# Christopher-Wang/DistriFlow

Measured on AMD Instinct MI355X. Metric: images/sec (whole node), MNIST CNN sync-SGD at 1/2/4/8 MI355X; async speedup, higher is better.
Workload: dtype bf16; 1 GPU; model=lenet5, global_batch=4096, per_gpu_batch=4096, parallelism=dp1, optimizer=sgd, graph=full, steps_per_graph=64, p2p_reason=single rank, step=train+reduce/update, params=61706

## Files before the change

csrc/bindings_fused.cpp:

```cpp
#include "bindings_comm.h"

namespace dfa_py {
namespace {

struct CPIn {
  const void* x = nullptr;
  int u8 = 0;
  const long long* idx = nullptr;
  long long nrows = 0;
};

CPIn cp_input(const torch::Tensor& x, const c10::optional<torch::Tensor>& idx, int64_t B, int64_t HWC) {
  CPIn r;
  TORCH_CHECK(x.is_cuda() && x.is_contiguous(), "x must be a contiguous GPU tensor");
  if (has(idx)) {
    need(*idx, at::kLong, "idx");
    TORCH_CHECK(idx->numel() >= B, "idx shorter than the batch");
    TORCH_CHECK(x.scalar_type() == at::kByte || x.scalar_type() == at::kBFloat16, "dataset must be u8 or bf16");
    TORCH_CHECK(x.dim() >= 1 && x.size(0) > 0 && x.numel() / x.size(0) == HWC, "dataset row size mismatch");
    TORCH_CHECK(x.scalar_type() == at::kByte, "indexed input must be a uint8 dataset");
    r.u8 = 1;
    r.idx = reinterpret_cast<const long long*>(idx->data_ptr<int64_t>());
    r.nrows = x.size(0);
  } else {
// ... 362 lines not shown
  need(labels, at::kInt, "lenet labels");
  TORCH_CHECK(labels.numel() >= (a.idx ? 1 : B), "lenet: labels too small");
  if (a.idx) a.nrows = std::min<int64_t>(a.nrows, labels.numel());
  a.labels = labels.data_ptr<int>();
  a.scale = (float)scale;
  const int64_t conv_n[4] = {150, 6, 2400, 16};
  for (int k = 0; k < 4; ++k) {
    need(conv[k], at::kFloat, "lenet conv param");
    need(conv_grads[k], at::kFloat, "lenet conv grad");
    TORCH_CHECK(conv[k].numel() == conv_n[k] && conv_grads[k].numel() == conv_n[k], "lenet: conv param size");
  }
  a.w1 = conv[0].data_ptr<float>();
  a.b1 = conv[1].data_ptr<float>();
  a.w2 = conv[2].data_ptr<float>();
  a.b2 = conv[3].data_ptr<float>();
  const int64_t NK[3][2] = {{120, 400}, {84, 120}, {10, 84}};
  const float* dw[3];
  const float* db[3];
  for (int l = 0; l < 3; ++l) {
    need(dense_w[l], at::kFloat, "lenet dense w");
    need(dense_b[l], at::kFloat, "lenet dense b");
    TORCH_CHECK(dense_w[l].numel() == NK[l][0] * NK[l][1], "lenet: dense ", l, " kernel must be [", NK[l][0], "][",
                NK[l][1], "]");
    TORCH_CHECK(dense_b[l].numel() == NK[l][0], "lenet: dense bias size");
    need(dense_gw[l], at::kFloat, "lenet dense gw");
    need(dense_gb[l], at::kFloat, "lenet dense gb");
    TORCH_CHECK(dense_gw[l].numel() == NK[l][0] * NK[l][1] && dense_gb[l].numel() == NK[l][0],
                "lenet: dense grad size");
    need(hT[l], at::kBFloat16, "lenet hT");
    need(dzT[l], at::kBFloat16, "lenet dzT");
    TORCH_CHECK(hT[l].dim() == 2 && hT[l].size(0) >= (NK[l][1] + 15) / 16 * 16 && hT[l].size(1) == lds,
                "lenet: hT must be [>= round16(K)][ldt]");
    TORCH_CHECK(dzT[l].dim() == 2 && dzT[l].size(0) >= (NK[l][0] + 15) / 16 * 16 && dzT[l].size(1) == lds,
                "lenet: dzT must be [>= round16(N)][ldt]");
    dw[l] = dense_w[l].data_ptr<float>();
    db[l] = dense_b[l].data_ptr<float>();
  }
  a.d1m = dw[0]; a.d2m = dw[1]; a.d3m = dw[2];
  a.d1b = db[0]; a.d2b = db[1]; a.d3b = db[2];
  const int nblk = dfa::lenet_blocks((int)B);
  need(conv_part, at::kFloat, "lenet conv_part");
  need(loss_part, at::kFloat, "lenet loss_part");
  need(stats, at::kFloat, "lenet stats");
  TORCH_CHECK(conv_part.numel() >= (int64_t)dfa::kLeNetConvStride * nblk, "lenet: conv_part too small");
  TORCH_CHECK(loss_part.numel() >= 2 * nblk && stats.numel() >= 2, "lenet: loss buffers too small");
  a.conv_part = conv_part.data_ptr<float>();
  a.loss_part = loss_part.data_ptr<float>();
  auto bp = [](torch::Tensor& t) { return reinterpret_cast<dfa::bf16*>(t.data_ptr()); };
  a.h0T = bp(hT[0]); a.h1T = bp(hT[1]); a.h2T = bp(hT[2]);
  a.dz1T = bp(dzT[0]); a.dz2T = bp(dzT[1]); a.dz3T = bp(dzT[2]);
  TORCH_CHECK(frag.is_cuda() && frag.is_contiguous() && (size_t)frag.nbytes() >= dfa::lenet_frag_bytes(),
              "lenet: fragment buffer too small");
  TORCH_CHECK(ftab.is_cuda() && ftab.scalar_type() == at::kByte && ftab.numel() == 98 * 2 * 16, "lenet: ftab");
  TORCH_CHECK(pxtab.is_cuda() && pxtab.scalar_type() == at::kShort && pxtab.numel() == 832, "lenet: pxtab");
  a.frag = frag.data_ptr();
  a.prep = prep ? 1 : 0;
  a.ftab = ftab.data_ptr<uint8_t>();
  a.pxtab = reinterpret_cast<const unsigned short*>(pxtab.data_ptr());
  a.B = (int)B;
  a.ldt = (int)lds;
  a.grad_scale = (float)grad_scale;
  dfa::LeNetRedArgs r{};
  r.kcols = (int)ldt;
  need(dense_part, at::kFloat, "lenet dense_part");
  TORCH_CHECK(dense_part.numel() >= dfa::lenet_dense_part_floats((int)B),
              "lenet: dense_part must hold lenet_dense_part_floats(B) zero-initialised floats");
  dfa::lenet_red_bind_scratch(dense_part.data_ptr<float>(), r);
  r.succ = red_succ ? 1 : 0;
  r.conv_part = a.conv_part;
  r.loss_part = a.loss_part;
  r.stats = stats.data_ptr<float>();
  r.g_w1 = conv_grads[0].data_ptr<float>();
  r.g_b1 = conv_grads[1].data_ptr<float>();
  r.g_w2 = conv_grads[2].data_ptr<float>();
  r.g_b2 = conv_grads[3].data_ptr<float>();
  for (int l = 0; l < 3; ++l) {
    r.L[l].dzT = reinterpret_cast<const dfa::bf16*>(dzT[l].data_ptr());
    r.L[l].hT = reinterpret_cast<const dfa::bf16*>(hT[l].data_ptr());
    r.L[l].gw = dense_gw[l].data_ptr<float>();
    r.L[l].gb = dense_gb[l].data_ptr<float>();
    r.L[l].N = (int)NK[l][0];
    r.L[l].K = (int)NK[l][1];
  }
  r.w1 = a.w1;
  r.w2 = a.w2;
  if (has(snap)) {
    need(*snap, at::kFloat, "lenet snap");
    TORCH_CHECK(snap->numel() >= 2 * 2550, "lenet: snap must hold 2 x 2550 floats");
    r.snap = snap->data_ptr<float>();
    TORCH_CHECK(conv_mom.empty() || conv_mom.size() == 2, "lenet: conv_mom = [m1, m2] or []");
    if (conv_mom.size() == 2) {
      need(conv_mom[0], at::kFloat, "lenet m1");
      need(conv_mom[1], at::kFloat, "lenet m2");
      TORCH_CHECK(conv_mom[0].numel() == 150 && conv_mom[1].numel() == 2400, "lenet: conv momentum sizes");
      r.m1 = conv_mom[0].data_ptr<float>();
      r.m2 = conv_mom[1].data_ptr<float>();
    }
  }
  if (has(sgd_master)) {
    need(*sgd_master, at::kFloat, "lenet sgd master");
    TORCH_CHECK(sgd_wbf.has_value() && sgd_hyper.has_value() && sgd_descs.has_value(),
                "lenet sgd: wbf, hyper and descs are required");
    need(*sgd_wbf, at::kBFloat16, "lenet sgd wbf");
    need(*sgd_hyper, at::kFloat, "lenet sgd hyper");
    TORCH_CHECK(sgd_hyper->numel() >= 5, "lenet sgd: hyper size");
    const torch::Tensor& dh = *sgd_descs;
    TORCH_CHECK(!dh.is_cuda() && dh.scalar_type() == at::kLong && dh.is_contiguous() &&
// ... 280 lines not shown
```

csrc/lenet_fused.hip:

```cpp
#include "common.h"
#include "diag.h"
#include "kernels.h"
#include "lenet_frag.h"
#include "ll_exchange.h"
#include "optim_device.h"
#include "ps_device.h"

#include <algorithm>
#include <cstdlib>
#include <type_traits>
#include <vector>

namespace dfa {
namespace {

constexpr int IMG = 8;
constexpr int NT = 512;
constexpr int NW = NT / 64;
constexpr int ccdiv(int a, int b) { return (a + b - 1) / b; }
constexpr int XS_ELEMS = IMG * 1024 + 32;
constexpr int OFF_XS = 0;
constexpr int OFF_P1 = OFF_XS + XS_ELEMS * 2;
constexpr int OFF_C1 = OFF_P1 + IMG * 196 * 16;
constexpr int DC2_RS = 104;
constexpr int NM = IMG * DC2_RS;
constexpr int OFF_K = OFF_C1 + IMG * 196 * 4;
constexpr int OFF_PX = OFF_K + 32;
constexpr int OFF_FT = OFF_PX + NM * 2;
constexpr int OFF_W = OFF_FT + 98 * 2 * 16;
constexpr int OFF_KZ = OFF_W + 128;
constexpr int OFF_U = OFF_KZ + 32;
constexpr int OFF_XS1 = OFF_U + 32;
constexpr int LD0 = 424, LD1 = 136, LD2 = 104, LD3 = 40;
constexpr int OFF_H0 = OFF_U;
constexpr int OFF_H1 = OFF_H0 + IMG * LD0 * 2;
constexpr int OFF_H2 = OFF_H1 + IMG * LD1 * 2;
constexpr int OFF_Z3 = OFF_H2 + IMG * LD2 * 2;
constexpr int OFF_Z2 = OFF_Z3 + IMG * LD3 * 2;
constexpr int OFF_Z1 = OFF_Z2 + IMG * LD2 * 2;
constexpr int OFF_ZR = OFF_Z1 + IMG * LD1 * 2;
constexpr int OFF_LG = OFF_ZR + LD0 * 2;
constexpr int OFF_C2 = OFF_LG + IMG * 16 * 4;
constexpr int U_DENSE = OFF_C2 + IMG * 25 * 16 - OFF_U;
constexpr int OFF_DC2 = OFF_U;
constexpr int U_DC2 = NM * 16 * 2;
constexpr int OFF_RED = OFF_XS1 + XS_ELEMS * 2;
constexpr int U_G = 32 + XS_ELEMS * 2 + 4 * 16 * 32 * 4;
__device__ __forceinline__ int dc2_swz(int t) { return t ^ ((t >> 3) & 7); }
constexpr int cmax(int a, int b) { return a > b ? a : b; }
constexpr int NFP1 = (FR_C2 - FR_C1) * 64, NFP2 = (FR_DG - FR_C2) * 64;
constexpr int OFF_FC1 = OFF_XS1;
constexpr int OFF_FC2 = OFF_U + U_DENSE;
constexpr int U_FC2 = U_DENSE + NFP2 * 16;
static_assert(FR_C1 == 0 && FR_C2 - FR_C1 == 15 && FR_DG - FR_C2 == 7, "phase 0 stages fragments 0 .. 21 as one range");
static_assert(OFF_FC1 + NFP1 * 16 <= OFF_XS1 + (XS_ELEMS / 8 - 1) * 16, "build_shift1 overwrites the conv1 fragments");
constexpr int OFF_DB = OFF_U + (cmax(cmax(cmax(U_DENSE, U_DC2), U_G), U_FC2) + 15) / 16 * 16;
constexpr int OFF_ST = OFF_DB + 864;
constexpr int LDS_BYTES = OFF_ST + 128;
static_assert(OFF_U == OFF_C1 + IMG * 196 * 4 + 128 + 98 * 2 * 16 + 800 * 2 + 128 && OFF_U % 16 == 0 && OFF_KZ % 16 == 0 && OFF_H1 % 16 == 0 && OFF_ZR % 16 == 0 && OFF_C2 % 16 == 0 && OFF_RED % 16 == 0 && OFF_DB % 16 == 0 && OFF_ST % 16 == 0 &&
                  OFF_PX % 16 == 0 && OFF_W % 16 == 0 && OFF_FC1 % 16 == 0 && OFF_FC2 % 16 == 0,
              "LDS carve must stay 16-byte aligned");
static_assert(2 * LDS_BYTES <= 160 * 1024, "two workgroups per CU");

typedef __bf16 bf16x4_vs __attribute__((__vector_size__(8)));

#define LN_STAMP(slot)                                                            \
  do {                                                                            \
    if (stamps) {                                                                 \
      __builtin_amdgcn_sched_barrier(0);                                          \
      unsigned long long t_;                                                      \
      asm volatile("s_memtime %0\n\ts_waitcnt lgkmcnt(0)" : "=s"(t_)::"memory"); \
      __builtin_amdgcn_sched_barrier(0);                                          \
      if (threadIdx.x == 0) STMP[(slot)] = t_;                                    \
    }                                                                             \
  } while (0)

template <int CTRL>
__device__ __forceinline__ float dpp_f(float v) {
  return __builtin_bit_cast(float, __builtin_amdgcn_update_dpp(0, __builtin_bit_cast(int, v), CTRL, 0xf, 0xf, false));
}
__device__ __forceinline__ float row16_max(float v) {
  v = fmaxf(v, dpp_f<0xB1>(v));
  v = fmaxf(v, dpp_f<0x4E>(v));
  v = fmaxf(v, dpp_f<0x141>(v));
  return fmaxf(v, dpp_f<0x140>(v));
}
__device__ __forceinline__ float row16_sum(float v) {
  v += dpp_f<0xB1>(v);
  v += dpp_f<0x4E>(v);
  v += dpp_f<0x141>(v);
  return v + dpp_f<0x140>(v);
}

__device__ __forceinline__ bf16x4 tr_read(const bf16* p) {
  auto* lp = (__attribute__((address_space(3))) bf16*)(const_cast<bf16*>(p));
  const bf16x4_vs v =
      __builtin_amdgcn_ds_read_tr16_b64_v4bf16(reinterpret_cast<__attribute__((address_space(3))) bf16x4_vs*>(lp));
  return __builtin_bit_cast(bf16x4, v);
}
__device__ __forceinline__ bf16x8 cat8(bf16x4 a, bf16x4 b) {
  bf16x8 r;
#pragma unroll
  for (int e = 0; e < 4; ++e) {
    r[e] = a[e];
    r[e + 4] = b[e];
  }
  return r;
}
__device__ __forceinline__ bf16x8 ld8(const bf16* p) { return *reinterpret_cast<const bf16x8*>(p); }
__device__ __forceinline__ void st8(bf16* p, const bf16x8& v) { *reinterpret_cast<bf16x8*>(p) = v; }
__device__ __forceinline__ bf16x8 zero8() {
// ... 130 lines not shown
    if (__hip_atomic_compare_exchange_strong(p.dlock + k, &free_, (unsigned)p.rank + 1u, __ATOMIC_RELAXED,
                                             __ATOMIC_RELAXED, __HIP_MEMORY_SCOPE_SYSTEM)) {
      P = __hip_atomic_load(p.pref + k, __ATOMIC_RELAXED, __HIP_MEMORY_SCOPE_SYSTEM);
      const unsigned* fl = ps_inbox_flags(p, k);
      while (n < R && n < 255u &&
             __hip_atomic_load(const_cast<unsigned*>(fl) + (P + n) % R, __ATOMIC_RELAXED, __HIP_MEMORY_SCOPE_SYSTEM) ==
                 P + n + 1u)
        ++n;
      if (n == 0) __hip_atomic_store(p.dlock + k, 0u, __ATOMIC_RELAXED, __HIP_MEMORY_SCOPE_SYSTEM);
      c = P + n;
    }
    __hip_atomic_store(ps_owner_drain_words(p) + k, ps_owner_word(ep, n, P), __ATOMIC_RELAXED, __HIP_MEMORY_SCOPE_AGENT);
    s_cnt[k] = c;
  }
  __syncthreads();
  if (threadIdx.x == 0) {
    unsigned cnt = 0xffffffffu;
    for (int j = 0; j < p.nshards; ++j) cnt = s_cnt[j] < cnt ? s_cnt[j] : cnt;
    const unsigned dec = __hip_atomic_load(p.scratch + kPSDecision, __ATOMIC_RELAXED, __HIP_MEMORY_SCOPE_AGENT) & 7u;
    if (dec == kPSAccept && cnt == p.scratch[kPSSeq]) cnt += 1u;
    if (dec == kPSAccept || dec == kPSReject) ps_note_refresh(p, cnt);
  }
}

__device__ __forceinline__ void lenet_ps_admission(const PSArgs& p, bool excl) {
  const long long bid = *p.bid_out;
  const unsigned applied0 = ps_read_applied(p);
  const unsigned ep = __hip_atomic_load(p.scratch + kPSEpoch, __ATOMIC_RELAXED, __HIP_MEMORY_SCOPE_AGENT) + 1u;
  const unsigned dec = ps_admit(p, false);
  const bool owner = p.owner_ring > 0;
  if (!owner && (dec == kPSAccept || dec == kPSReject)) ps_note_refresh(p, applied0 + (dec == kPSAccept ? 1u : 0u));
  __hip_atomic_store(p.scratch + kPSDecision, (ep << 3) | dec, __ATOMIC_RELAXED, __HIP_MEMORY_SCOPE_AGENT);
  if (excl) {
    __hip_atomic_store(p.scratch + kPSEpoch, ep, __ATOMIC_RELAXED, __HIP_MEMORY_SCOPE_AGENT);
    if (dec == kPSAccept) ps_publish_applied(p);
  }
  if (dec == kPSAccept && p.done_epoch != nullptr) complete_microbatch(p, bid);
}

template <bool TRIM>
__global__ void __launch_bounds__(NT, 2 * NT / 256) lenet_train_kernel(LeNetArgs a) {
  if ((int)blockIdx.x >= a.nblk) {
    if (a.ps_admit && threadIdx.x == 0) lenet_ps_admission(a.ps, a.ps_excl != 0);
    return;
  }
  extern __shared__ __attribute__((aligned(16))) char smem[];
  bf16* Xs = reinterpret_cast<bf16*>(smem + OFF_XS);
  bf16* Xs1 = reinterpret_cast<bf16*>(smem + OFF_XS1);
  bf16* P1 = reinterpret_cast<bf16*>(smem + OFF_P1);
  unsigned* C1 = reinterpret_cast<unsigned*>(smem + OFF_C1);
  bf16* KO = reinterpret_cast<bf16*>(smem + OFF_K);
  unsigned char* FT = reinterpret_cast<unsigned char*>(smem + OFF_FT);
  unsigned short* PX = reinterpret_cast<unsigned short*>(smem + OFF_PX);
  float* WS = reinterpret_cast<float*>(smem + OFF_W);
  bf16* H0 = reinterpret_cast<bf16*>(smem + OFF_H0);
  bf16* H1 = reinterpret_cast<bf16*>(smem + OFF_H1);
  bf16* H2 = reinterpret_cast<bf16*>(smem + OFF_H2);
  bf16* Z3 = reinterpret_cast<bf16*>(smem + OFF_Z3);
  bf16* Z2 = reinterpret_cast<bf16*>(smem + OFF_Z2);
  bf16* Z1 = reinterpret_cast<bf16*>(smem + OFF_Z1);
  bf16* ZR = reinterpret_cast<bf16*>(smem + OFF_ZR);
  float* LG = reinterpret_cast<float*>(smem + OFF_LG);
  unsigned char* C2 = reinterpret_cast<unsigned char*>(smem + OFF_C2);
  bf16* DC2 = reinterpret_cast<bf16*>(smem + OFF_DC2);
  float* RED = reinterpret_cast<float*>(smem + OFF_RED);

  const int tid = threadIdx.x, lane = tid & 63, w = __builtin_amdgcn_readfirstlane(tid >> 6), i = lane & 15,
            g = lane >> 4;
  const int r0 = lenet_img_group(blockIdx.x, a.nblk) * (TRIM ? a.ipw : IMG);
  const int rows = min(TRIM ? a.ipw : IMG, a.B - r0);
  const int nA = TRIM ? 2 * ((7 * rows + 1) / 2) : 56;
  const int nB = TRIM ? (13 * rows + 1) / 2 : NM / 16;
  const int nE = TRIM ? (13 * rows + 3) / 4 : NM / 32;
  const int nF = TRIM ? (49 * rows + 7) / 8 : 49;
  const int nG = TRIM ? 14 * rows : IMG * 14;
  const bf16x8* __restrict__ frag = reinterpret_cast<const bf16x8*>(a.frag);
  float* part = a.conv_part + (long long)blockIdx.x * kLeNetConvStride;
  unsigned long long* const stamps = a.stamps;
  unsigned long long* const STMP = reinterpret_cast<unsigned long long*>(smem + OFF_ST);
  LN_STAMP(0);

  const int ximg = tid / 28, xrow = tid - 28 * (tid / 28);
  const bool xload = tid < IMG * 28 && ximg < rows;
  const bool lload = tid >= 256 && tid < 256 + IMG && tid - 256 < rows;
  long long xsrc = 0, lsrc = 0;
  if (xload) xsrc = a.idx ? a.idx[r0 + ximg] : (long long)(r0 + ximg);
  if (lload) lsrc = a.idx ? a.idx[r0 + tid - 256] : (long long)(r0 + tid - 256);
  uint4 tabv = {0u, 0u, 0u, 0u};
  if (tid < 98 * 2) tabv = reinterpret_cast<const uint4*>(a.ftab)[tid];
  else if (tid >= 264 && tid < 264 + NM / 8) tabv = reinterpret_cast<const uint4*>(a.pxtab)[tid - 264];
  static_assert(98 * 2 <= 256 && 264 + NM / 8 <= 448 && 448 + 22 <= NT, "phase 0 staging thread ranges");
  float biasv = 0.f, dbv = 0.f;
  if (tid >= 448 && tid < 448 + 22) biasv = *(tid < 454 ? a.b1 + (tid - 448) : a.b2 + (tid - 454));
  if (tid < 214) dbv = *(tid < 120 ? a.d1b + tid : (tid < 204 ? a.d2b + (tid - 120) : a.d3b + (tid - 204)));
  constexpr int NFK = ccdiv(NFP1 + NFP2, NT);
  bf16x8 fv[NFK];
#pragma unroll
  for (int k = 0; k < NFK; ++k) fv[k] = frag[FR_C1 * 64 + min(tid + NT * k, NFP1 + NFP2 - 1)];
  const int lbl = a.labels[lsrc < 0 ? 0 : (lsrc >= a.nrows ? a.nrows - 1 : lsrc)];
  unsigned xv[14];
  {
    const long long src = xsrc < 0 ? 0 : (xsrc >= a.nrows ? a.nrows - 1 : xsrc);
    const int xr = xload ? xrow : 0;
    if (a.x_u8 != nullptr) {
      const unsigned* p = reinterpret_cast<const unsigned*>(a.x_u8 + src * 784 + xr * 28);
#pragma unroll
      for (int k = 0; k < 7; ++k) xv[k] = p[k];
    } else {
      const uint2* p = reinterpret_cast<const uint2*>(a.x_bf + src * 784 + xr * 28);
#pragma unroll
      for (int k = 0; k < 7; ++k) {
        const uint2 v = p[k];
        xv[2 * k] = v.x;
        xv[2 * k + 1] = v.y;
      }
    }
  }
  const bf16x8 z8 = zero8();
  bf16x8 one6 = z8;
  one6[6] = (bf16)1.f;
  for (int e = tid; e < (OFF_K - OFF_XS) / 16; e += NT)
    st8(Xs + 8 * e, (e >= OFF_P1 / 16 && e < OFF_C1 / 16) ? one6 : z8);
  static_assert(OFF_FC2 + NFP2 * 16 == OFF_DB, "the conv2 fragment image ends the union");
  if (tid < (OFF_FC1 - OFF_U) / 16) st8(reinterpret_cast<bf16*>(smem + OFF_U) + 8 * tid, z8);
  for (int e = (OFF_FC1 - OFF_U) / 16 + NFP1 + tid; e < (OFF_FC2 - OFF_U) / 16; e += NT)
    st8(reinterpret_cast<bf16*>(smem + OFF_U) + 8 * e, z8);
#pragma unroll
  for (int k = 0; k < NFK; ++k) {
    const int p = tid + NT * k;
    if (p < NFP1) st8(reinterpret_cast<bf16*>(smem + OFF_FC1) + 8 * p, fv[k]);
    else if (p < NFP1 + NFP2) st8(reinterpret_cast<bf16*>(smem + OFF_FC2) + 8 * (p - NFP1), fv[k]);
  }
  if (tid < 2) {
    bf16x8 o;
#pragma unroll
    for (int e = 0; e < 8; ++e) o[e] = (bf16)1.f;
    st8(KO + 8 * tid, o);
  } else if (tid < 4) {
    st8(reinterpret_cast<bf16*>(smem + OFF_KZ) + 8 * (tid - 2), z8);
  }
  if (tid < 98 * 2) reinterpret_cast<uint4*>(FT)[tid] = tabv;
  else if (tid >= 264 && tid < 264 + NM / 8) reinterpret_cast<uint4*>(PX)[tid - 264] = tabv;
  if (tid >= 448 && tid < 448 + 22) WS[tid - 448] = biasv;
  float* DB = reinterpret_cast<float*>(smem + OFF_DB);
  if (tid < 214) DB[tid] = dbv;
  int* LBL = reinterpret_cast<int*>(WS + 24);
  if (tid >= 256 && tid < 256 + IMG) LBL[tid - 256] = lbl;
  __syncthreads();
  bf16x8 bc[15];
#pragma unroll
  for (int f = 0; f < 15; ++f) bc[f] = ld8(reinterpret_cast<const bf16*>(smem + OFF_FC1) + 8 * (f * 64 + lane));
  if (xload) {
    unsigned* dst = reinterpret_cast<unsigned*>(Xs + ximg * 1024 + (xrow + 2) * 32 + 2);
    if (a.x_u8 != nullptr) {
#pragma unroll
      for (int k = 0; k < 7; ++k)
#pragma unroll
        for (int h = 0; h < 2; ++h) {
          const float f0 = (float)((xv[k] >> (16 * h)) & 255u) * a.scale;
          const float f1 = (float)((xv[k] >> (16 * h + 8)) & 255u) * a.scale;
          const unsigned lo = __builtin_bit_cast(unsigned short, f2bf(f0));
          const unsigned hi = __builtin_bit_cast(unsigned short, f2bf(f1));
          dst[2 * k + h] = lo | (hi << 16);
        }
    } else {
#pragma unroll
      for (int k = 0; k < 14; ++k) dst[k] = xv[k];
    }
  }
  __syncthreads();
  build_shift1(Xs, Xs1);
  __syncthreads();
  LN_STAMP(1);

  {
    const float b1c[3] = {WS[(i >> 3)], WS[2 + (i >> 3)], WS[4 + (i >> 3)]};
#pragma unroll 2
    for (int u = w; u < nA; u += NT / 64) {
      const int mt = u >> 1, x0 = (u & 1) * 16;
      const int m = 16 * mt + i;
      const int img = m / 56, rem = m - 56 * (m / 56);
      const bf16* abase = ((rem & 1) ? Xs1 : Xs) + img * 1024 + (rem >> 1) * 32 + x0 + 8 * g;
      f32x4 acc[3];
#pragma unroll
      for (int T = 0; T < 3; ++T) acc[T] = {0.f, 0.f, 0.f, 0.f};
#pragma unroll
      for (int ky = 0; ky < 5; ++ky) {
        const bf16x8 av = ld8(abase + ky * 32);
#pragma unroll
        for (int T = 0; T < 3; ++T) acc[T] = mfma16x16x32(av, bc[ky * 3 + T], acc[T]);
      }
      const int m0 = 16 * mt + 4 * g;
      const int imgo = m0 / 56, py = (m0 - 56 * (m0 / 56)) >> 2;
      const int px = (x0 >> 1) + (i & 7);
      unsigned cw = 0;
#pragma unroll
      for (int T = 0; T < 3; ++T) {
        float best;
        unsigned code;
        pool4(acc[T][0] + b1c[T], acc[T][1] + b1c[T], acc[T][2] + b1c[T], acc[T][3] + b1c[T], best, code);
        const int c = 2 * T + (i >> 3);
        if (px < 14) P1[((imgo * 14 + py) * 14 + px) * 8 + c] = f2bf(best);
        cw |= code << (3 * c);
      }
      cw |= __shfl_xor(cw, 8, 64);
      if (i < 8 && px < 14) C1[(imgo * 14 + py) * 14 + px] = cw;
    }
  }
  __syncthreads();
  LN_STAMP(2);

  bf16x8 bw[7];
#pragma unroll
  for (int s = 0; s < 7; ++s) bw[s] = ld8(reinterpret_cast<const bf16*>(smem + OFF_FC2) + 8 * (s * 64 + lane));
  DenseFrags<13, ccdiv(8, NW)> f1;
  dense_load(f1, frag + FR_D1W * 64, 8);
  {
    int toff[7];
#pragma unroll
    for (int s = 0; s < 7; ++s) {
      const int tap = 4 * s + g;
      toff[s] = tap < 25 ? ((tap / 5) * 14 + (tap - 5 * (tap / 5))) * 8 : 0;
    }
    const float b2 = WS[6 + i];
#pragma unroll 2
    for (int mt = w; mt < nB; mt += NT / 64) {
      const bf16* abase = P1 + (int)PX[16 * mt + i] * 8;
      f32x4 acc = {0.f, 0.f, 0.f, 0.f};
#pragma unroll
      for (int s = 0; s < 7; ++s) acc = mfma16x16x32(ld8(abase + toff[s]), bw[s], acc);
      const int m0 = 16 * mt + 4 * g;
      const int img0 = m0 / DC2_RS, win0 = (m0 - DC2_RS * img0) >> 2;
      float best;
      unsigned code;
      pool4(acc[0] + b2, acc[1] + b2, acc[2] + b2, acc[3] + b2, best, code);
      if (win0 < 25) {
        H0[img0 * LD0 + win0 * 16 + i] = f2bf(best);
        C2[(img0 * 25 + win0) * 16 + i] = (unsigned char)code;
      }
    }
  }
  __syncthreads();
  LN_STAMP(3);

  for (int k = tid; k < 400; k += NT) {
    if (rows == IMG) {
      bf16x8 v;
#pragma unroll
      for (int r = 0; r < IMG; ++r) v[r] = H0[r * LD0 + k];
      st8(a.h0T + lenet_act_pos(k, r0, a.ldt), v);
    } else {
      for (int r = 0; r < rows; ++r) a.h0T[lenet_act_pos(k, r0 + r, a.ldt)] = H0[r * LD0 + k];
    }
  }
  DenseFrags<4, ccdiv(6, NW)> f2;
  DenseFrags<3, 1> f3;
  dense_load(f2, frag + FR_D2W * 64, 6);
  dense_load(f3, frag + FR_D3W * 64, 1);
  dense_fwd(f1, H0, LD0, ZR, DB, 120, true, H1, LD1, nullptr, a.h1T, a.ldt, r0, rows);
  __syncthreads();
  DenseFrags<1, ccdiv(6, NW)> g3;
  DenseFrags<3, ccdiv(8, NW)> g2;
  dense_load(g3, frag + FR_D3WT * 64, 6);
  dense_load(g2, frag + FR_D2WT * 64, 8);
  dense_fwd(f2, H1, LD1, ZR, DB + 120, 84, true, H2, LD2, nullptr, a.h2T, a.ldt, r0, rows);
  __syncthreads();
  dense_fwd(f3, H2, LD2, ZR, DB + 204, 10, false, nullptr, 0, LG, nullptr, a.ldt, r0, rows);
  __syncthreads();
  LN_STAMP(4);
  if (tid < IMG * 16) {
    const int r = tid >> 4, c = tid & 15;
    const bool live = r < rows;
    const int y = min(max(LBL[r], 0), 9);
    const float z = c < 10 ? LG[r * 16 + c] : -INFINITY;
    if (a.logits && live && c < 10) a.logits[(long long)(r0 + r) * 10 + c] = z;
    const float mx = row16_max(z);
    const unsigned long long hit = __ballot(z == mx);
    const int am = __builtin_ctzll((hit >> (16 * (r & 3))) | 0x10000ull);
    const float e = c < 10 ? __expf(z - mx) : 0.f;
    const float ssum = row16_sum(e);
    if (c < 10) {
      const float gv = live ? (e * (1.f / ssum) - (c == y ? 1.f : 0.f)) * a.grad_scale : 0.f;
      Z3[r * LD3 + c] = f2bf(gv);
      if (live) a.dz3T[lenet_act_pos(c, r0 + r, a.ldt)] = f2bf(gv);
    }
    if (c == y) LG[r * 16 + 14] = live ? -(z - mx - __logf(ssum)) : 0.f;
    if (c == 15) LG[r * 16 + 15] = (live && am == y) ? 1.f : 0.f;
  }
  __syncthreads();
  if (tid == 0) {
    float ls = 0.f, cs = 0.f;
#pragma unroll
    for (int r = 0; r < IMG; ++r) {
      ls += LG[r * 16 + 14];
      cs += LG[r * 16 + 15];
    }
    a.loss_part[2 * blockIdx.x] = ls;
    a.loss_part[2 * blockIdx.x + 1] = cs;
  }
  DenseFrags<4, ccdiv(25, NW)> g1;
  dense_load(g1, frag + FR_D1WT * 64, 25);
  __syncthreads();
  LN_STAMP(5);
  dense_bwd(g3, Z3, LD3, ZR, 84, H2, LD2, Z2, LD2, a.dz2T, a.ldt, r0, rows);
  __syncthreads();
  dense_bwd(g2, Z2, LD2, ZR, 120, H1, LD1, Z1, LD1, a.dz1T, a.ldt, r0, rows);
  __syncthreads();
  dense_bwd(g1, Z1, LD1, ZR, 400, H0, LD0, H0, LD0, nullptr, 0, r0, rows);
  __syncthreads();
  LN_STAMP(6);

  {
    bf16x8 dp[2];
    unsigned long long cd[2];
#pragma unroll
    for (int k = 0; k < 2; ++k) {
      const int it = tid + k * NT;
      if (it < IMG * 50) {
        const int img = it / 50, rem = it - 50 * (it / 50), win = rem >> 1, nh = rem & 1;
        dp[k] = ld8(H0 + img * LD0 + win * 16 + 8 * nh);
        cd[k] = *reinterpret_cast<const unsigned long long*>(C2 + (img * 25 + win) * 16 + 8 * nh);
      }
    }
    __syncthreads();
#pragma unroll
    for (int k = 0; k < 2; ++k) {
      const int it = tid + k * NT;
      if (it < IMG * 50) {
        const int img = it / 50, rem = it - 50 * (it / 50), win = rem >> 1, nh = rem & 1;
#pragma unroll
        for (int d = 0; d < 4; ++d) {
          bf16x8 o;
#pragma unroll
          for (int e = 0; e < 8; ++e) o[e] = ((cd[k] >> (8 * e)) & 255u) == (unsigned)d ? dp[k][e] : (bf16)0.f;
          st8(DC2 + ((img * DC2_RS + dc2_swz(win * 4 + d)) * 16 + 8 * nh), o);
        }
      }
    }
  }
  if (tid < IMG * 8) {
    const int img = tid >> 3, rr = (tid >> 1) & 3, nh = tid & 1;
    st8(DC2 + ((img * DC2_RS + dc2_swz(100 + rr)) * 16 + 8 * nh), zero8());
  }
  __syncthreads();
  LN_STAMP(7);

  bf16x8 bd[15];
#pragma unroll
  for (int s = 0; s < 15; ++s) bd[s] = frag[(FR_DG + s) * 64 + lane];
  {
    const int q = (lane & 15) >> 2, p = lane & 3;
    const int h = w >> 2, cg = w & 3;
    constexpr int KTM = ccdiv(13, NW / 2);
    static_assert(NW == 8 && KTM == 4, "phase E: 2 K-halves x 4 column groups of 4, 3, 3, 3 tiles");
    const int nlo = (nE + 1) >> 1;
    const int sb = h ? nlo : 0, se = h ? nE : nlo;
    const int ntile = cg == 0 ? KTM : KTM - 1;
    f32x4 acc[KTM];
#pragma unroll
    for (int k = 0; k < KTM; ++k) acc[k] = {0.f, 0.f, 0.f, 0.f};
    auto ldAv = [&](int s) -> bf16x8 {
      const int mA = 32 * s + 8 * g + q;
      const int b = 4 * s + g, sx = (b - 13 * ((b * 79) >> 10)) & 7;
      return cat8(tr_read(DC2 + (mA ^ sx) * 16 + 4 * p), tr_read(DC2 + ((mA + 4) ^ sx) * 16 + 4 * p));
    };
    const unsigned short* pxl = PX + 8 * g + q;
    auto run = [&](auto ktc) {
      constexpr int KT = decltype(ktc)::value;
      int toff[KT];
#pragma unroll
      for (int k = 0; k < KT; ++k) {
        const int tap = 2 * (cg + NW / 2 * k) + (p >> 1);
        toff[k] = tap < 25 ? ((tap / 5) * 14 + (tap - 5 * (tap / 5))) * 8 + 4 * (p & 1) : 4 * (p & 1);
      }
      auto step = [&](const bf16x8& av, unsigned px0, unsigned px1) {
        const bf16* pb0 = P1 + 8 * px0;
        const bf16* pb1 = P1 + 8 * px1;
        bf16x4 t0[KT], t1[KT];
#pragma unroll
        for (int k = 0; k < KT; ++k) {
          t0[k] = tr_read(pb0 + toff[k]);
          t1[k] = tr_read(pb1 + toff[k]);
        }
#pragma unroll
        for (int k = 0; k < KT; ++k) acc[k] = mfma16x16x32(av, cat8(t0[k], t1[k]), acc[k]);
      };
      bf16x8 ava = ldAv(sb);
      unsigned pxa0 = pxl[32 * sb], pxa1 = pxl[32 * sb + 4];
      int s = sb;
#pragma unroll 1
      for (; s + 1 < se; s += 2) {
        const bf16x8 avb = ldAv(s + 1);
        const unsigned pxb0 = pxl[32 * (s + 1)], pxb1 = pxl[32 * (s + 1) + 4];
        __builtin_amdgcn_sched_barrier(0);
        step(ava, pxa0, pxa1);
        __builtin_amdgcn_sched_barrier(0);
        const int sn = s + 2 < se ? s + 2 : s;
        ava = ldAv(sn);
        pxa0 = pxl[32 * sn];
        pxa1 = pxl[32 * sn + 4];
        __builtin_amdgcn_sched_barrier(0);
        step(avb, pxb0, pxb1);
        __builtin_amdgcn_sched_barrier(0);
      }
      if (s < se) step(ava, pxa0, pxa1);
    };
    if (cg == 0) run(std::integral_constant<int, KTM>{});
    else run(std::integral_constant<int, KTM - 1>{});
    static_assert(13 * 64 * 16 <= IMG * 196 * 16, "the upper half's 13 accumulator tiles fit in P1");
    f32x4* ES = reinterpret_cast<f32x4*>(smem + OFF_P1);
    __syncthreads();
    if (h) {
#pragma unroll
      for (int k = 0; k < KTM; ++k)
        if (k < ntile) ES[(cg + NW / 2 * k) * 64 + lane] = acc[k];
    }
    __syncthreads();
    if (!h) {
#pragma unroll
      for (int k = 0; k < KTM; ++k) {
        if (k < ntile) {
          const int T = cg + NW / 2 * k;
          const f32x4 up = ES[T * 64 + lane];
          const int tap = 2 * T + (i >> 3), c = i & 7;
#pragma unroll
          for (int r = 0; r < 4; ++r) {
            const int n = 4 * g + r;
            const float v = acc[k][r] + up[r];
            if (tap < 25 && c < 6) part[(long long)(kLeNetPW2 + n * 150 + tap * 6 + c)] = v;
            else if (tap == 0 && c == 6) part[(long long)(kLeNetPB2 + n)] = v;
          }
        }
      }
    }
  }
  __syncthreads();
  LN_STAMP(8);

  {
    const int bcol = i >> 3, c = i & 7;
#pragma unroll 2
    for (int mt = w; mt < nF; mt += NT / 64) {
      const int m = 16 * mt + i;
      const int img = m / 98, rem = m - 98 * (m / 98);
      const uint4 tv = *reinterpret_cast<const uint4*>(FT + (rem * 2 + (g >> 1)) * 16);
      const unsigned tw[4] = {tv.x, tv.y, tv.z, tv.w};
      const unsigned dbase = (unsigned)OFF_DC2 + 16u * (unsigned)(g & 1) + 32u * (unsigned)(img * DC2_RS);
      auto ldA = [&](int st) -> bf16x8 {
        const unsigned t = (tw[st >> 2] >> (8 * (st & 3))) & 255u;
        return *reinterpret_cast<const bf16x8*>(smem + dbase + 32u * t);
      };
      f32x4 acc = {0.f, 0.f, 0.f, 0.f};
      bf16x8 a0 = ldA(0), a1 = ldA(1), a2 = ldA(2);
#pragma unroll
      for (int s = 0; s < 15; ++s) {
        acc = mfma16x16x32(a0, bd[s], acc);
        a0 = a1;
        a1 = a2;
        if (s + 3 < 15) a2 = ldA(s + 3);
      }
      if (c < 6) {
#pragma unroll
        for (int r = 0; r < 4; ++r) {
          const int mm = 16 * mt + 4 * g + r;
          P1[(2 * mm + bcol) * 8 + c] = f2bf(acc[r]);
        }
      }
    }
  }
  __syncthreads();
  build_shift1(Xs, Xs1);
  __syncthreads();
  LN_STAMP(9);

  {
    f32x4 acc[2] = {{0.f, 0.f, 0.f, 0.f}, {0.f, 0.f, 0.f, 0.f}};
    const int gdy = i >= 6 && i < 12 ? 1 : 0;
    const int ca = i < 6 ? i : (i < 12 ? i - 6 : 5);
    constexpr int kXs1 = (OFF_XS1 - OFF_XS) / 2;
    unsigned boff[2], bconst[2];
    bool breal[2];
#pragma unroll
    for (int T = 0; T < 2; ++T) {
      const int e = 16 * T + i;
      const int ep = e < 30 ? e : 0;
      const int ky = ep / 5, kx = ep - 5 * (ep / 5);
      boff[T] = 2u * (unsigned)(((kx & 1) ? kXs1 : 0) + ky * 32 + 8 * g + 2 * (kx >> 1));
      breal[T] = e < 30;
      bconst[T] = e == 30 ? (unsigned)OFF_K : (unsigned)OFF_KZ;
    }
    unsigned cmask[4];
#pragma unroll
    for (int wd = 0; wd < 4; ++wd) cmask[wd] = (4 * g + wd < 14 && i < 12) ? 0u : 8u;
#pragma unroll 2
    for (int rp = w; rp < nG; rp += NT / 64) {
      const int img = rp / 14, py = rp - 14 * (rp / 14);
      const int p0 = (img * 14 + py) * 14 + 4 * g;
      const uint2 cA = *reinterpret_cast<const uint2*>(C1 + p0);
      const uint2 cB = *reinterpret_cast<const uint2*>(C1 + p0 + 2);
      const unsigned cw[4] = {cA.x, cA.y, cB.x, cB.y};
      unsigned aw[4];
#pragma unroll
      for (int wd = 0; wd < 4; ++wd) {
        const unsigned sel = (((cw[wd] >> (3 * ca)) & 7u) | cmask[wd]) - 2u * (unsigned)gdy;
        const unsigned pv = *reinterpret_cast<const unsigned short*>(P1 + (p0 + wd) * 8 + ca);
        aw[wd] = sel < 2u ? pv << (sel << 4) : 0u;
      }
      const bf16x8 av = __builtin_bit_cast(bf16x8, uint4{aw[0], aw[1], aw[2], aw[3]});
      const unsigned rowb = (unsigned)OFF_XS + 2u * (unsigned)(img * 1024 + 2 * py * 32);
#pragma unroll
      for (int T = 0; T < 2; ++T) {
        const unsigned* bp = reinterpret_cast<const unsigned*>(smem + (breal[T] ? rowb + boff[T] : bconst[T]));
        const bf16x8 bv = __builtin_bit_cast(bf16x8, uint4{bp[0], bp[1], bp[2], bp[3]});
        acc[T] = mfma16x16x32(av, bv, acc[T]);
      }
    }
    if (w >= 4) {
// ... 1214 lines not shown
```

distriflow_amd/ops/__init__.py:

```python
from __future__ import annotations

import torch

from .. import native
from ..diagnostics import on as _diag_on
from . import reference as ref

MODE_DIRECT, MODE_FWD, MODE_DGRAD = 0, 1, 2


class _DebugSync:

    def __init__(self, mod):
        self._mod = mod

    def __getattr__(self, name):
        fn = getattr(self._mod, name)
        if not callable(fn) or isinstance(fn, type):
            return fn

        def wrapped(*args, **kw):
            out = fn(*args, **kw)
            if torch.cuda.is_available() and not torch.cuda.is_current_stream_capturing():
                try:
# ... 782 lines not shown
    tt = target if idx is None else target.index_select(0, idx.long().clamp(0, target.shape[0] - 1))
    tt = tt[:B]
    if dense:
        t = tt.float()
        ref_class = t.argmax(1)
    else:
        ref_class = tt.long().view(-1).clamp(0, C - 1)
        t = torch.nn.functional.one_hot(ref_class, C).float()
    p = torch.softmax(z, dim=1) if act == 1 else (torch.sigmoid(z) if act == 2 else z)
    terms, g = _loss_terms(kind, p, t)
    if dlogits is not None:
        dz = p * (g - (g * p).sum(1, keepdim=True)) if act == 1 else (g * p * (1 - p) if act == 2 else g)
        dlogits[:, :C].copy_((dz * grad_scale).to(dlogits.dtype))
    if stats is not None:
        stats[0] += terms.sum()
        stats[1] += (z.argmax(1) == ref_class).float().sum()
    return stats


def classifier_metrics(z, labels, loss: str, softmax, out):
    if z.is_cuda:
        out_act = 2 if softmax == "sigmoid" else (1 if softmax in (True, "softmax") else 0)
        _C().classifier_metrics(z.contiguous(), labels.to(torch.int32).contiguous(), METRIC_KINDS[loss], out_act,
                                out)
        return out
    from ..losses import accuracy, get_loss

    if softmax == "sigmoid":
        p = torch.sigmoid(z.float())
    else:
        p = torch.softmax(z.float(), dim=1) if softmax in (True, "softmax") else z.float()
    onehot = torch.nn.functional.one_hot(labels.long(), z.shape[1]).float()
    out[0] = get_loss(loss)(onehot, p).sum()
    out[1] = accuracy(labels, p).sum()
    return out


def lenet_supported() -> bool:
    m = native.get(build_if_missing=False)
    return m is not None and hasattr(m, "lenet_train")


def lenet_frag_bytes() -> int:
    return int(_C().lenet_frag_bytes())


def lenet_blocks(B: int) -> int:
    return int(_C().lenet_blocks(int(B)))


_LENET_TABLES = {}


def lenet_tables(device):
    key = str(device)
    if key not in _LENET_TABLES:
        import numpy as np

        swz = lambda t: t ^ ((t >> 3) & 7)
        ft = np.full((98, 2, 16), swz(100), dtype=np.uint8)
        for yx in range(98):
            y, X2 = divmod(yx, 7)
            for hf in range(2):
                for s in range(16):
                    P = 2 * s + hf
                    if P >= 30:
                        continue
                    ky, u = divmod(P, 6)
                    oy, ox = y - ky, 2 * X2 + 1 - u
                    if 0 <= oy < 10 and 0 <= ox < 10:
                        ft[yx, hf, s] = swz((((oy >> 1) * 5 + (ox >> 1)) << 2) + ((oy & 1) << 1) + (ox & 1))
        px = np.zeros(832, dtype=np.int16)
        for m in range(832):
            img, q = divmod(m, 104)
            if q >= 100:
                px[m] = img * 196
                continue
            win, d = divmod(q, 4)
            py, pxx = divmod(win, 5)
            px[m] = img * 196 + (2 * py + (d >> 1)) * 14 + 2 * pxx + (d & 1)
        nbytes = int(_C().lenet_frag_bytes())
        _LENET_TABLES[key] = (torch.from_numpy(ft.reshape(-1)).to(device), torch.from_numpy(px).to(device),
                              torch.zeros(nbytes, dtype=torch.uint8, device=device))
    return _LENET_TABLES[key]


def lenet_dense_part_floats(B: int) -> int:
    return int(_C().lenet_dense_part_floats(int(B)))


def lenet_train(x, labels, conv, dense_w, dense_b, conv_grads, dense_gw, dense_gb, hT, dzT, conv_part,
                dense_part, loss_part, stats, grad_scale, frag=None, prep=True, snap=None, conv_mom=(), sgd=None):
    if isinstance(x, GatherRef):
        src, idx, scale = x.data, x.idx, x.scale
    else:
        src, idx, scale = x.contiguous(), None, 1.0
    if isinstance(labels, LabelRef):
        lab, lidx = labels.labels, labels.idx
        if idx is None:
            idx = lidx
    else:
        lab = labels if labels.dtype == torch.int32 else labels.to(torch.int32)
    B = x.shape[0]
    ftab, pxtab, scratch = lenet_tables(stats.device)
    _C().lenet_train(src, idx, float(scale), lab, list(conv), list(dense_w), list(dense_b),
                     list(conv_grads), list(dense_gw), list(dense_gb), list(hT), list(dzT), conv_part, dense_part,
                     loss_part, stats, scratch if frag is None else frag, ftab, pxtab, int(B), float(grad_scale),
                     prep=bool(prep) or frag is None, snap=snap, conv_mom=list(conv_mom),
                     red_succ=_diag_on("lenet_succ"), **(sgd or {}))


def lenet_red_error(dense_part) -> int:
    o = int(_C().lenet_red_err_offset())
    return int(dense_part[o:o + 1].view(torch.int32)[0].item())


def convpool_plan(H, W, C, KH, KW, pad, N, B=0, ws_floats=0) -> dict:
    return _C().convpool_plan(H, W, C, KH, KW, pad, N, B=B, ws_floats=ws_floats)


def convpool_supported(H, W, C, KH, KW, pad, N) -> bool:
    return native.get(build_if_missing=False) is not None and convpool_plan(H, W, C, KH, KW, pad, N)["ok"]


def convpool_fwd_layout(H, W, C, KH, KW, pad, N):
    return tuple(convpool_plan(H, W, C, KH, KW, pad, N)[k] for k in ("Cp", "Kpad2", "pair"))


def convpool_dgrad_layout(H, W, C, KH, KW, pad, N):
    return tuple(convpool_plan(H, W, C, KH, KW, pad, N)[k] for k in ("dgrad_pair", "K2pad"))


def _cp_in(x):
# ... 63 lines not shown
```

Before: 83.42 million images/s.

## Replace dC2 XOR swizzle with class-based row placement tables for bank-conflict-free LDS access

```diff
diff --git a/csrc/bindings_fused.cpp b/csrc/bindings_fused.cpp
--- a/csrc/bindings_fused.cpp
+++ b/csrc/bindings_fused.cpp
@@ -438,7 +438,7 @@
   TORCH_CHECK(frag.is_cuda() && frag.is_contiguous() && (size_t)frag.nbytes() >= dfa::lenet_frag_bytes(),
               "lenet: fragment buffer too small");
   TORCH_CHECK(ftab.is_cuda() && ftab.scalar_type() == at::kByte && ftab.numel() == 98 * 2 * 16, "lenet: ftab");
-  TORCH_CHECK(pxtab.is_cuda() && pxtab.scalar_type() == at::kShort && pxtab.numel() == 832, "lenet: pxtab");
+  TORCH_CHECK(pxtab.is_cuda() && pxtab.scalar_type() == at::kShort && pxtab.numel() == 832 + 104, "lenet: pxtab");
   a.frag = frag.data_ptr();
   a.prep = prep ? 1 : 0;
   a.ftab = ftab.data_ptr<uint8_t>();
diff --git a/csrc/lenet_fused.hip b/csrc/lenet_fused.hip
--- a/csrc/lenet_fused.hip
+++ b/csrc/lenet_fused.hip
@@ -46,7 +46,6 @@
 constexpr int U_DC2 = NM * 16 * 2;
 constexpr int OFF_RED = OFF_XS1 + XS_ELEMS * 2;
 constexpr int U_G = 32 + XS_ELEMS * 2 + 4 * 16 * 32 * 4;
-__device__ __forceinline__ int dc2_swz(int t) { return t ^ ((t >> 3) & 7); }
 constexpr int cmax(int a, int b) { return a > b ? a : b; }
 constexpr int NFP1 = (FR_C2 - FR_C1) * 64, NFP2 = (FR_DG - FR_C2) * 64;
 constexpr int OFF_FC1 = OFF_XS1;
@@ -56,7 +55,10 @@
 static_assert(OFF_FC1 + NFP1 * 16 <= OFF_XS1 + (XS_ELEMS / 8 - 1) * 16, "build_shift1 overwrites the conv1 fragments");
 constexpr int OFF_DB = OFF_U + (cmax(cmax(cmax(U_DENSE, U_DC2), U_G), U_FC2) + 15) / 16 * 16;
 constexpr int OFF_ST = OFF_DB + 864;
-constexpr int LDS_BYTES = OFF_ST + 128;
+constexpr int OFF_RT = OFF_ST + 128;
+constexpr int OFF_ZB = OFF_DC2 + (OFF_RT + DC2_RS * 2 - OFF_DC2 + 255) / 256 * 256;
+constexpr int LDS_BYTES = OFF_ZB + 256;
+static_assert(OFF_RT % 16 == 0 && (OFF_ZB - OFF_DC2) % 256 == 0 && (DC2_RS * 32) % 256 == 0, "dC2 row classes");
 static_assert(OFF_U == OFF_C1 + IMG * 196 * 4 + 128 + 98 * 2 * 16 + 800 * 2 + 128 && OFF_U % 16 == 0 && OFF_KZ % 16 == 0 && OFF_H1 % 16 == 0 && OFF_ZR % 16 == 0 && OFF_C2 % 16 == 0 && OFF_RED % 16 == 0 && OFF_DB % 16 == 0 && OFF_ST % 16 == 0 &&
                   OFF_PX % 16 == 0 && OFF_W % 16 == 0 && OFF_FC1 % 16 == 0 && OFF_FC2 % 16 == 0,
               "LDS carve must stay 16-byte aligned");
@@ -293,6 +295,9 @@
   bf16* KO = reinterpret_cast<bf16*>(smem + OFF_K);
   unsigned char* FT = reinterpret_cast<unsigned char*>(smem + OFF_FT);
   unsigned short* PX = reinterpret_cast<unsigned short*>(smem + OFF_PX);
+  unsigned short* RT = reinterpret_cast<unsigned short*>(smem + OFF_RT);
+  constexpr int NPXV = (NM + DC2_RS) / 8;
+  static_assert((NM + DC2_RS) % 8 == 0 && NM % 8 == 0, "pxtab pieces");
   float* WS = reinterpret_cast<float*>(smem + OFF_W);
   bf16* H0 = reinterpret_cast<bf16*>(smem + OFF_H0);
   bf16* H1 = reinterpret_cast<bf16*>(smem + OFF_H1);
@@ -329,8 +334,8 @@
   if (lload) lsrc = a.idx ? a.idx[r0 + tid - 256] : (long long)(r0 + tid - 256);
   uint4 tabv = {0u, 0u, 0u, 0u};
   if (tid < 98 * 2) tabv = reinterpret_cast<const uint4*>(a.ftab)[tid];
-  else if (tid >= 264 && tid < 264 + NM / 8) tabv = reinterpret_cast<const uint4*>(a.pxtab)[tid - 264];
-  static_assert(98 * 2 <= 256 && 264 + NM / 8 <= 448 && 448 + 22 <= NT, "phase 0 staging thread ranges");
+  else if (tid >= 264 && tid < 264 + NPXV) tabv = reinterpret_cast<const uint4*>(a.pxtab)[tid - 264];
+  static_assert(98 * 2 <= 256 && 264 + NPXV <= 448 && 448 + 22 <= NT, "phase 0 staging thread ranges");
   float biasv = 0.f, dbv = 0.f;
   if (tid >= 448 && tid < 448 + 22) biasv = *(tid < 454 ? a.b1 + (tid - 448) : a.b2 + (tid - 454));
   if (tid < 214) dbv = *(tid < 120 ? a.d1b + tid : (tid < 204 ? a.d2b + (tid - 120) : a.d3b + (tid - 204)));
@@ -382,6 +387,8 @@
   }
   if (tid < 98 * 2) reinterpret_cast<uint4*>(FT)[tid] = tabv;
   else if (tid >= 264 && tid < 264 + NM / 8) reinterpret_cast<uint4*>(PX)[tid - 264] = tabv;
+  else if (tid >= 264 + NM / 8 && tid < 264 + NPXV) reinterpret_cast<uint4*>(RT)[tid - 264 - NM / 8] = tabv;
+  if (tid >= 480 && tid < 480 + 16) st8(reinterpret_cast<bf16*>(smem + OFF_ZB) + 8 * (tid - 480), z8);
   if (tid >= 448 && tid < 448 + 22) WS[tid - 448] = biasv;
   float* DB = reinterpret_cast<float*>(smem + OFF_DB);
   if (tid < 214) DB[tid] = dbv;
@@ -466,7 +473,8 @@
     const float b2 = WS[6 + i];
 #pragma unroll 2
     for (int mt = w; mt < nB; mt += NT / 64) {
-      const bf16* abase = P1 + (int)PX[16 * mt + i] * 8;
+      const int m = 16 * mt + i, img = ((m >> 3) * 79) >> 10;
+      const bf16* abase = P1 + (img * 196 + (int)(RT[m - DC2_RS * img] & 255u)) * 8;
       f32x4 acc = {0.f, 0.f, 0.f, 0.f};
 #pragma unroll
       for (int s = 0; s < 7; ++s) acc = mfma16x16x32(ld8(abase + toff[s]), bw[s], acc);
@@ -554,6 +562,7 @@
   {
     bf16x8 dp[2];
     unsigned long long cd[2];
+    uint2 pl[2];
 #pragma unroll
     for (int k = 0; k < 2; ++k) {
       const int it = tid + k * NT;
@@ -561,27 +570,31 @@
         const int img = it / 50, rem = it - 50 * (it / 50), win = rem >> 1, nh = rem & 1;
         dp[k] = ld8(H0 + img * LD0 + win * 16 + 8 * nh);
         cd[k] = *reinterpret_cast<const unsigned long long*>(C2 + (img * 25 + win) * 16 + 8 * nh);
-      }
-    }
+        pl[k] = *reinterpret_cast<const uint2*>(RT + win * 4);
+      }
+    }
+    const unsigned zrow = RT[100 + ((tid >> 1) & 3)] >> 8;
     __syncthreads();
 #pragma unroll
     for (int k = 0; k < 2; ++k) {
       const int it = tid + k * NT;
       if (it < IMG * 50) {
         const int img = it / 50, rem = it - 50 * (it / 50), win = rem >> 1, nh = rem & 1;
+        const unsigned plw[2] = {pl[k].x, pl[k].y};
 #pragma unroll
         for (int d = 0; d < 4; ++d) {
           bf16x8 o;
 #pragma unroll
           for (int e = 0; e < 8; ++e) o[e] = ((cd[k] >> (8 * e)) & 255u) == (unsigned)d ? dp[k][e] : (bf16)0.f;
-          st8(DC2 + ((img * DC2_RS + dc2_swz(win * 4 + d)) * 16 + 8 * nh), o);
+          const int row = (int)((plw[d >> 1] >> (16 * (d & 1) + 8)) & 255u);
+          st8(DC2 + ((img * DC2_RS + row) * 16 + 8 * nh), o);
         }
       }
     }
-  }
-  if (tid < IMG * 8) {
-    const int img = tid >> 3, rr = (tid >> 1) & 3, nh = tid & 1;
-    st8(DC2 + ((img * DC2_RS + dc2_swz(100 + rr)) * 16 + 8 * nh), zero8());
+    if (tid < IMG * 8) {
+      const int img = tid >> 3, nh = tid & 1;
+      st8(DC2 + ((img * DC2_RS + (int)zrow) * 16 + 8 * nh), zero8());
+    }
   }
   __syncthreads();
   LN_STAMP(7);
@@ -601,11 +614,10 @@
 #pragma unroll
     for (int k = 0; k < KTM; ++k) acc[k] = {0.f, 0.f, 0.f, 0.f};
     auto ldAv = [&](int s) -> bf16x8 {
-      const int mA = 32 * s + 8 * g + q;
-      const int b = 4 * s + g, sx = (b - 13 * ((b * 79) >> 10)) & 7;
-      return cat8(tr_read(DC2 + (mA ^ sx) * 16 + 4 * p), tr_read(DC2 + ((mA + 4) ^ sx) * 16 + 4 * p));
+      const int mA = 32 * s + 4 * g + q;
+      return cat8(tr_read(DC2 + mA * 16 + 4 * p), tr_read(DC2 + (mA + 16) * 16 + 4 * p));
     };
-    const unsigned short* pxl = PX + 8 * g + q;
+    const unsigned short* pxl = PX + 4 * g + q;
     auto run = [&](auto ktc) {
       constexpr int KT = decltype(ktc)::value;
       int toff[KT];
@@ -627,19 +639,19 @@
         for (int k = 0; k < KT; ++k) acc[k] = mfma16x16x32(av, cat8(t0[k], t1[k]), acc[k]);
       };
       bf16x8 ava = ldAv(sb);
-      unsigned pxa0 = pxl[32 * sb], pxa1 = pxl[32 * sb + 4];
+      unsigned pxa0 = pxl[32 * sb], pxa1 = pxl[32 * sb + 16];
       int s = sb;
 #pragma unroll 1
       for (; s + 1 < se; s += 2) {
         const bf16x8 avb = ldAv(s + 1);
-        const unsigned pxb0 = pxl[32 * (s + 1)], pxb1 = pxl[32 * (s + 1) + 4];
+        const unsigned pxb0 = pxl[32 * (s + 1)], pxb1 = pxl[32 * (s + 1) + 16];
         __builtin_amdgcn_sched_barrier(0);
         step(ava, pxa0, pxa1);
         __builtin_amdgcn_sched_barrier(0);
         const int sn = s + 2 < se ? s + 2 : s;
         ava = ldAv(sn);
         pxa0 = pxl[32 * sn];
-        pxa1 = pxl[32 * sn + 4];
+        pxa1 = pxl[32 * sn + 16];
         __builtin_amdgcn_sched_barrier(0);
         step(avb, pxb0, pxb1);
         __builtin_amdgcn_sched_barrier(0);
@@ -680,16 +692,20 @@
 
   {
     const int bcol = i >> 3, c = i & 7;
+    const int ip = i < 4 ? i : (i < 12 ? i + 4 : i - 8);
+    const int gp = (0x1320 >> (4 * g)) & 3;
 #pragma unroll 2
     for (int mt = w; mt < nF; mt += NT / 64) {
-      const int m = 16 * mt + i;
+      const int m = 16 * mt + ip;
       const int img = m / 98, rem = m - 98 * (m / 98);
       const uint4 tv = *reinterpret_cast<const uint4*>(FT + (rem * 2 + (g >> 1)) * 16);
       const unsigned tw[4] = {tv.x, tv.y, tv.z, tv.w};
       const unsigned dbase = (unsigned)OFF_DC2 + 16u * (unsigned)(g & 1) + 32u * (unsigned)(img * DC2_RS);
+      const unsigned zdelta = (unsigned)(OFF_ZB - OFF_DC2 - 32 * 128) - 32u * (unsigned)(img * DC2_RS);
       auto ldA = [&](int st) -> bf16x8 {
         const unsigned t = (tw[st >> 2] >> (8 * (st & 3))) & 255u;
-        return *reinterpret_cast<const bf16x8*>(smem + dbase + 32u * t);
+        const unsigned zm = 0u - ((tw[st >> 2] >> (8 * (st & 3) + 7)) & 1u);
+        return *reinterpret_cast<const bf16x8*>(smem + dbase + 32u * t + (zm & zdelta));
       };
       f32x4 acc = {0.f, 0.f, 0.f, 0.f};
       bf16x8 a0 = ldA(0), a1 = ldA(1), a2 = ldA(2);
@@ -703,7 +719,7 @@
       if (c < 6) {
 #pragma unroll
         for (int r = 0; r < 4; ++r) {
-          const int mm = 16 * mt + 4 * g + r;
+          const int mm = 16 * mt + 4 * gp + r;
           P1[(2 * mm + bcol) * 8 + c] = f2bf(acc[r]);
         }
       }
diff --git a/distriflow_amd/ops/__init__.py b/distriflow_amd/ops/__init__.py
--- a/distriflow_amd/ops/__init__.py
+++ b/distriflow_amd/ops/__init__.py
@@ -858,33 +858,53 @@
 _LENET_TABLES = {}
 
 
+def lenet_dc2_class(oy: int, ox: int) -> int:
+    return ((ox >> 1) + 7 * oy + 4 * (ox & 1)) % 8
+
+
+def lenet_conv2_tables():
+    import numpy as np
+
+    pos = {}
+    for oy in range(10):
+        for ox in range(10):
+            pos[(((oy >> 1) * 5 + (ox >> 1)) << 2) + ((oy & 1) << 1) + (ox & 1)] = (oy, ox)
+    place = np.full(104, -1, dtype=np.int64)
+    fill = [0] * 8
+    for t in range(100):
+        c = lenet_dc2_class(*pos[t])
+        place[t] = c + 8 * fill[c]
+        fill[c] += 1
+    assert max(fill) <= 13
+    place[100:] = sorted(set(range(104)) - set(place[:100].tolist()))
+    winpix = np.zeros(104, dtype=np.int64)
+    for t, (oy, ox) in pos.items():
+        winpix[t] = oy * 14 + ox
+    rowpix = np.zeros(104, dtype=np.int64)
+    rowpix[place] = winpix
+    ft = np.zeros((98, 2, 16), dtype=np.uint8)
+    for yx in range(98):
+        y, X2 = divmod(yx, 7)
+        for hf in range(2):
+            for s in range(16):
+                ky, u = divmod(2 * s + hf, 6)
+                oy, ox = y - ky, 2 * X2 + 1 - u
+                if ky < 5 and 0 <= oy < 10 and 0 <= ox < 10:
+                    t = (((oy >> 1) * 5 + (ox >> 1)) << 2) + ((oy & 1) << 1) + (ox & 1)
+                    ft[yx, hf, s] = place[t]
+                else:
+                    ft[yx, hf, s] = 128 + lenet_dc2_class(oy, ox)
+    return place, ft, rowpix, winpix
+
+
 def lenet_tables(device):
     key = str(device)
     if key not in _LENET_TABLES:
         import numpy as np
 
-        swz = lambda t: t ^ ((t >> 3) & 7)
-        ft = np.full((98, 2, 16), swz(100), dtype=np.uint8)
-        for yx in range(98):
-            y, X2 = divmod(yx, 7)
-            for hf in range(2):
-                for s in range(16):
-                    P = 2 * s + hf
-                    if P >= 30:
-                        continue
-                    ky, u = divmod(P, 6)
-                    oy, ox = y - ky, 2 * X2 + 1 - u
-                    if 0 <= oy < 10 and 0 <= ox < 10:
-                        ft[yx, hf, s] = swz((((oy >> 1) * 5 + (ox >> 1)) << 2) + ((oy & 1) << 1) + (ox & 1))
-        px = np.zeros(832, dtype=np.int16)
-        for m in range(832):
-            img, q = divmod(m, 104)
-            if q >= 100:
-                px[m] = img * 196
-                continue
-            win, d = divmod(q, 4)
-            py, pxx = divmod(win, 5)
-            px[m] = img * 196 + (2 * py + (d >> 1)) * 14 + 2 * pxx + (d & 1)
+        place, ft, rowpix, winpix = lenet_conv2_tables()
+        px = np.concatenate([(np.arange(8)[:, None] * 196 + rowpix[None, :]).reshape(-1),
+                             winpix | (place << 8)]).astype(np.int16)
         nbytes = int(_C().lenet_frag_bytes())
         _LENET_TABLES[key] = (torch.from_numpy(ft.reshape(-1)).to(device), torch.from_numpy(px).to(device),
                               torch.zeros(nbytes, dtype=torch.uint8, device=device))
```

New measurement: 84.45 million images/s, median of 6. 1.01x the previous value.
